# LunaJang/Metabuli_work

Measured on AMD Instinct MI355X. Metric: reads/sec classified (150bp & 10kb) vs GTDB-scale DB at 1/2/4/8 MI355X, higher is better.
Workload: dtype u64

## Files before the change

metabuli_work_amd/classifier.py:

```python
from __future__ import annotations

import ctypes
import dataclasses
import gzip
import os
from typing import Iterator, List, Optional, Tuple

import numpy as np

from . import _abi
from ._abi import KMER_DTYPE, MATCH_DTYPE, RESULT_DTYPE, TAXCNT_DTYPE, MtbParams, ptr
from ._lib import MtbError, check, lib


@dataclasses.dataclass
class LocalParameters:
    seqMode: int = 2
    kmerFormat: int = 1
    syncmer: int = 0
    smerLen: int = 5
    reducedAA: int = 0
    skipRedundancy: int = 0
    minScore: float = 0.0
    minSpScore: float = 0.0
# ... 176 lines not shown
            o1 = off1[lo:hi + 1]
            o2 = off2[lo:hi + 1] if off2 is not None else None
            self.classify_batch(seq1, o1, seq2, o2, device_input=device_input, fetch=False)
            rec = torch.empty((hi - lo, _abi.RESULT_DTYPE.itemsize), dtype=torch.uint8, device=dev)
            self.copy_results(rec.data_ptr(), on_device=True)
            pool = torch.empty((max(self.n_taxcnt(), 1), _abi.TAXCNT_DTYPE.itemsize), dtype=torch.uint8, device=dev)
            nt = self.copy_taxcnt(pool.data_ptr(), on_device=True)
            q, m = self.last_counts()
            recs.append(rec)
            pools.append(pool[:nt])
            qk, mm = qk + q, mm + m
            st = self.stats()
            stats = st if stats is None else {k: (max(stats[k], v) if k == "max_read_matches" else
                                                  v if k in ("join_path", "uniform_units") else stats[k] + v)
                                              for k, v in st.items()}
            stage += self.stage_ms()
            kern += self.kernel_ms()
        recs[1].view(torch.int32).view(-1, _abi.RESULT_DTYPE.itemsize // 4)[:, 4] += pools[0].shape[0]
        torch.cuda.synchronize(dev)
        self._dev_batch = _DevBatch(torch.cat(recs), torch.cat(pools), qk, mm, stats, stage, kern)

    def _classify_halves(self, seq1, off1, seq2, off2, n, device_input) -> BatchResult:
        mid = n // 2
        parts = []
        for lo, hi in ((0, mid), (mid, n)):
            o1 = off1[lo:hi + 1]
            o2 = off2[lo:hi + 1] if off2 is not None else None
            parts.append(self.classify_batch(seq1, o1, seq2, o2, device_input=device_input))
        a, b = parts
        rb = b.results.copy()
        rb["taxcnt_offset"] += len(a.taxcnt)
        return BatchResult(np.concatenate([a.results, rb]), np.concatenate([a.taxcnt, b.taxcnt]),
                           a.query_kmers + b.query_kmers, a.matches + b.matches, a.stage_ms + b.stage_ms)

    def taxcnt(self) -> np.ndarray:
        if getattr(self, "_dev_batch", None) is not None:
            return self._dev_batch.taxcnt.cpu().numpy().reshape(-1).view(TAXCNT_DTYPE).copy()
        nt = ctypes.c_uint64(0)
        lib().mtb_get_taxcnt(self.handle, ctypes.c_void_p(0), 0, ctypes.byref(nt))
        tc = np.zeros(int(nt.value), TAXCNT_DTYPE)
        check(lib().mtb_get_taxcnt(self.handle, ptr(tc), len(tc), ctypes.byref(nt)), "mtb_get_taxcnt")
        return tc

    def last_counts(self) -> Tuple[int, int]:
        if getattr(self, "_dev_batch", None) is not None:
            return self._dev_batch.query_kmers, self._dev_batch.matches
        q, m = ctypes.c_uint64(0), ctypes.c_uint64(0)
        lib().mtb_last_counts(self.handle, ctypes.byref(q), ctypes.byref(m))
        return int(q.value), int(m.value)

    STATS = ["slots", "query_kmers", "matched_queries", "matches", "max_read_matches", "groups", "groups_ge2",
             "species_runs", "wave_runs", "wave_runs_emulated", "join_path", "live_matches", "gallop_queries",
             "spilled_matches", "long_run_queries", "filter_reruns", "db_records_read", "dup_aa_queries",
             "dup_key_queries", "uniform_units"]

    def stats(self) -> dict:
        if getattr(self, "_dev_batch", None) is not None:
            return dict(self._dev_batch.stats)
        out = (ctypes.c_uint64 * len(self.STATS))()
        lib().mtb_last_stats(self.handle, out, len(self.STATS))
        return {k: int(v) for k, v in zip(self.STATS, out)}

    def stage_ms(self) -> np.ndarray:
        if getattr(self, "_dev_batch", None) is not None:
            return self._dev_batch.stage_ms.copy()
        ms = (ctypes.c_float * 5)()
        lib().mtb_last_stage_ms(self.handle, ms, 5)
        return np.array(list(ms), np.float32)

    def kernel_ms(self) -> np.ndarray:
        if getattr(self, "_dev_batch", None) is not None:
            return self._dev_batch.kernel_ms.copy()
        ms = (ctypes.c_float * 7)()
        lib().mtb_last_kernel_ms(self.handle, ms, 7)
        return np.array(list(ms), np.float32)

    def _copy_dev(self, t, dst_ptr: int, on_device: bool) -> None:
        import torch

        del on_device
        if t.numel():
            torch.cuda.synchronize(t.device)
            check(lib().mtb_memcpy(ctypes.c_void_p(dst_ptr), ctypes.c_void_p(t.data_ptr()), t.numel()), "mtb_memcpy")

    def copy_results(self, dst_ptr: int, on_device: bool = True) -> None:
        if getattr(self, "_dev_batch", None) is not None:
            return self._copy_dev(self._dev_batch.results, dst_ptr, on_device)
        check(lib().mtb_copy_results(self.handle, ctypes.c_void_p(dst_ptr), int(on_device)), "mtb_copy_results")

    def n_taxcnt(self) -> int:
        if getattr(self, "_dev_batch", None) is not None:
            return int(self._dev_batch.taxcnt.shape[0])
        nt = ctypes.c_uint64(0)
        lib().mtb_get_taxcnt(self.handle, ctypes.c_void_p(0), 0, ctypes.byref(nt))
        return int(nt.value)

    def copy_taxcnt(self, dst_ptr: int, on_device: bool = True) -> int:
        if getattr(self, "_dev_batch", None) is not None:
            self._copy_dev(self._dev_batch.taxcnt, dst_ptr, on_device)
            return int(self._dev_batch.taxcnt.shape[0])
        nt = ctypes.c_uint64(0)
        check(lib().mtb_copy_taxcnt(self.handle, ctypes.c_void_p(dst_ptr), int(on_device), ctypes.byref(nt)),
              "mtb_copy_taxcnt")
        return int(nt.value)

    def query_kmers(self) -> np.ndarray:
        q = self.stats()["query_kmers"]
# ... 216 lines not shown
```

metabuli_work_amd/csrc/mtb_api.hip:

```cpp
#include <chrono>
#include <cmath>
#include <cstdio>
#include <cstring>
#include <string>
#include <vector>
#include <algorithm>
#include <memory>
#include <charconv>
#include <mutex>
#include <unordered_map>

#include "mtb_host.h"
#include "mtb_launch.h"
#include <cstdlib>

using namespace mtb;

#define HIP_TRY(x)                                                                                   \
    do {                                                                                             \
        hipError_t e_ = (x);                                                                         \
        if (e_ != hipSuccess) {                                                                      \
            set_error(std::string("HIP error ") + hipGetErrorString(e_) + " at " #x);                 \
            return e_ == hipErrorOutOfMemory ? MTB_ERR_OOM : MTB_ERR_HIP;                            \
        }                                                                                            \
// ... 110 lines not shown
    uint64_t binRcForce = 0;
    bool binDigits = true;
    bool uniformUnits = true;
    uint32_t upr = 0;
    uint64_t binHost[kSortBins] = {};
    bool noFilter = false;
    uint32_t spillShift = 0;
    bool sparse = false;
    uint32_t maxW = 0;
    uint32_t maxMate = 0;
    int sortLoFine = kQuerySortLoFine;
    bool forceGeneric = false;
    bool segsortGlobal = false;
    uint32_t mergeSeg = 0;
    int waveTaxon = -1;
    int emulateAll = 0;
    bool pruneCompact = true;
    bool noAlias = false;
    uint64_t aliasBytes = 0;
    int32_t* spOf = nullptr;
    int32_t maxTax = 0;
    int32_t *tNodeOf = nullptr, *tNodeTax = nullptr, *tParent = nullptr, *tDepth = nullptr, *tSpParent = nullptr;
    uint8_t* tFlags = nullptr;
    uint32_t cladePerMatch = 2;
    std::vector<int32_t> hNodeOf;
    std::vector<std::string> hRank;
    HostTaxonomy hTax;
    mutable std::vector<std::string> lineage;
    mutable std::once_flag lineageOnce;
    std::shared_ptr<void> pipelineCache;
    mutable mtb::TaxText taxText;
    mutable std::once_flag taxTextOnce;
    WsBudget ws;
    DevBuf seq1, off1, seq2, off2, meta, reserve, slotOff, qlen, scanTmp;
    DevBuf keysA, valsA, keysB, valsB, radixCounts, radixOffs;
    DevBuf readCnt, mOff, matches, matchesSorted, segScratch, maxSeg, errFlag;
    DevBuf ordKA, ordVA, ordKB, ordVB, matchWin, unitRead, unitInfo, mStage, mRank, mTotal, mDirect, ovFlag, waveList, waveCount, devStats;
    DevBuf qFrom, probeStats;
    DevBuf longList, longCnt;
    DevBuf qStart;
    uint32_t longCap = 0;
    DevBuf chunkIn, chunkCnt, chunkSrcOff;
    DevBuf liveCnt, liveOff;
    DevBuf runFlag, runCnt, runScan;
    DevBuf segLen;
    DevBuf sizeLists;
    DevBuf digA, digB;
    DevBuf binCnt, binTab;
    DevBuf maskOut1, maskOut2, maskProb, maskScale;
    DevBuf readLens;
    DevBuf readCnt64;
    uint64_t liveM = 0;
    double openS[8] = {0, 0, 0, 0, 0, 0, 0, 0};
    static constexpr int kNumStats = 20;
    uint64_t stats[kNumStats] = {};
    uint32_t chunkC = 1;
    uint64_t stageRegion = 0;
    uint64_t spillCap = 0;
    DevBuf emMap, emCnt, emScratch, emPacked, emCnt32, emOff;
    bool emValid = false;
    bool emPackedValid = false;
    std::vector<mtb_em_map> emHost;
    std::vector<uint32_t> spKmers;
    std::string dbDir;
    DevBuf local, paths, comb, conn, spScore, spKeep,
        pathCnt, gStart, sStart, runGroup, clade, tcPool, tcLen, tcOff, tcOut, results;
    uint32_t nReads = 0;
    uint64_t Q = 0, M = 0, nTaxcnt = 0;
    uint64_t Qall = 0;
    double presentShare = 0.5;
    const uint64_t* qKeys = nullptr;
    const uint32_t* qSlots = nullptr;
    bool keepStages = false;
    bool probed = false;
    bool matchOnly = false;
    float stageMs[5] = {0, 0, 0, 0, 0};
    hipEvent_t ev[6]{};
    static constexpr int kNumKern = 7;
    float kernMs[kNumKern] = {0, 0, 0, 0, 0, 0, 0};
    hipEvent_t kev[2 * kNumKern]{};
};

static std::vector<DevBuf*> batch_bufs(mtb_ctx* c);

static void bind_workspace(mtb_ctx* c, size_t cap) {
    c->ws.cap = cap;
    if (const char* e = getenv("MTB_WORKSPACE_CAP")) {
        char* end = nullptr;
        double v = strtod(e, &end);
        const char u = end ? *end : 0;
        v *= u == 'G' || u == 'g' ? 1e9 : u == 'M' || u == 'm' ? 1e6 : u == 'K' || u == 'k' ? 1e3 : 1.0;
        c->ws.cap = v > 0 ? (size_t)v : 0;
    }
    for (DevBuf* b : batch_bufs(c)) b->budget = &c->ws;
}

static void free_db(mtb_ctx* c) {
    if (c->dbArrays) {
        c->dbArrays.reset();
        c->db = nullptr;
        c->dirMem = nullptr;
        c->lines = nullptr;
        c->lineP = nullptr;
        c->runOff = nullptr;
        c->lineExt = nullptr;
        c->link = nullptr;
        return;
// ... 1251 lines not shown
    const uint32_t maxW = metaMax[0];
    c->maxMate = metaMax[1];
    const uint32_t C = std::min<uint32_t>(std::max<uint32_t>(maxW, 1), 64);
    c->maxW = maxW;
    c->upr = c->uniformUnits && maxW <= 64 ? (paired ? 12u : 6u) : 0u;
    c->stats[19] = c->upr;
    launch_read_units(c->meta.as<ReadMeta>(), n, C, c->upr, c->reserve.as<uint32_t>(), s);
    exclusive_scan_u32(c->reserve.as<uint32_t>(), n, c->slotOff.as<uint64_t>(), c->scanTmp.p, s);
    uint64_t U = 0;
    HIP_TRY(hipMemcpyAsync(&U, c->slotOff.as<uint64_t>() + n, sizeof(uint64_t), hipMemcpyDeviceToHost, s));
    HIP_TRY(hipStreamSynchronize(s));
    HIP_TRY(c->unitRead.ensure(sizeof(uint32_t) * std::max<uint64_t>(U, 1)));
    launch_unit_read(c->slotOff.as<uint64_t>(), n, c->unitRead.as<uint32_t>(), s);
    const uint64_t R = extract_slots(U, C);
    const uint64_t Rc = std::max<uint64_t>(R, 1);
    if (R >= 0xFFFFFFFFull) { set_error("batch has >= 2^32 k-mer slots: split it"); return MTB_ERR_ARG; }
    c->chunkC = C;
    c->stats[0] = R;
    c->stats[15] = 0;
    HIP_TRY(c->unitInfo.ensure(16 * std::max<uint64_t>(U, 1)));
    HIP_TRY(c->errFlag.ensure(sizeof(int)));
    HIP_TRY(hipMemsetAsync(c->errFlag.p, 0, sizeof(int), s));
    HIP_TRY(c->mOff.ensure(sizeof(uint64_t) * (n + 1)));
    c->probed = !c->forceGeneric && c->joinMode == 2;
    c->stats[10] = c->probed ? 0 : 1;
    c->matchOnly = (flags & MTB_MATCH_ONLY) != 0;
    int jrc = join_stage(c, dSeq1, dOff1, dSeq2, dOff2, n, U, C, R, Rc);
    if (jrc != MTB_OK) return jrc;
    if (c->matchOnly) {
        for (int k = 10; k < 14; k++) HIP_TRY(hipEventRecord(c->kev[k], s));
        c->nTaxcnt = 0;
    } else {
        int rc = assign_stage(c, n, c->keepStages);
        if (rc != MTB_OK) return rc;
    }
    HIP_TRY(hipEventRecord(c->ev[4], s));
    HIP_TRY(hipGetLastError());
    int err = 0;
    unsigned long long dstat[4] = {0, 0, 0, 0};
    HIP_TRY(hipMemcpyAsync(&err, c->errFlag.p, sizeof(int), hipMemcpyDeviceToHost, s));
    HIP_TRY(hipMemcpyAsync(dstat, c->devStats.p, sizeof(dstat), hipMemcpyDeviceToHost, s));
    if (results && !c->matchOnly)
        HIP_TRY(hipMemcpyAsync(results, c->results.p, sizeof(mtb_result) * n, hipMemcpyDeviceToHost, s));
    HIP_TRY(hipStreamSynchronize(s));
    c->stats[9] = dstat[1];
    {
        std::vector<unsigned long long> ps(kProbeStatsLen);
        HIP_TRY(hipMemcpy(ps.data(), c->probeStats.p, sizeof(unsigned long long) * ps.size(), hipMemcpyDeviceToHost));
        c->stats[2] = 0;
        for (uint32_t i = 0; i < kStatStripes; i++) c->stats[2] += ps[i];
        c->stats[12] = ps[kStatStripes];
        c->stats[16] = 0;
        for (uint32_t i = 0; i < kStatStripes; i++) c->stats[16] += ps[kStatStripes + 1 + i];
    }
    for (int k = 0; k < 4; k++) HIP_TRY(hipEventElapsedTime(&c->stageMs[k], c->ev[k], c->ev[k + 1]));
    HIP_TRY(hipEventElapsedTime(&c->stageMs[4], c->ev[0], c->ev[4]));
    for (int k = 0; k < mtb_ctx::kNumKern; k++)
        HIP_TRY(hipEventElapsedTime(&c->kernMs[k], c->kev[2 * k], c->kev[2 * k + 1]));
    if (const char* e = getenv("MTB_WS_REPORT"); e && atoi(e)) {
        const std::vector<DevBuf*> bufs = batch_bufs(c);
        const char* const* names = batch_buf_names();
        std::vector<std::pair<uint64_t, const char*>> big;
        for (size_t i = 0; i < bufs.size(); i++)
            if (bufs[i]->bytes >= (256ull << 20)) big.push_back({bufs[i]->bytes, names[i]});
        std::sort(big.begin(), big.end(), [](auto& a, auto& b) { return a.first > b.first; });
        fprintf(stderr, "[mtb ws] %u reads, Q %llu, M %llu, live %llu: workspace %.2f GB (K6 scratch aliased %.2f GB):",
                n, (unsigned long long)c->Q, (unsigned long long)c->M, (unsigned long long)c->liveM,
                ctx_workspace_bytes(c) / 1e9, c->aliasBytes / 1e9);
        for (auto& b : big) fprintf(stderr, " %s %.2f", b.second, b.first / 1e9);
        fprintf(stderr, "\n");
    }
    return err ? batch_error(err) : MTB_OK;
}

int mtb_classify_batch(mtb_ctx* c, const char* seq, const uint64_t* off, const char* seq2, const uint64_t* off2,
                       uint32_t n, uint32_t flags, mtb_result* results) {
    const int rc = classify_batch(c, seq, off, seq2, off2, n, flags, results);
    if (rc != MTB_ERR_OOM) return rc;
    (void)hipGetLastError();
    const double held = c->ws.used * 1e-9;
    mtb::ctx_release_workspace(c);
    char msg[200];
    snprintf(msg, sizeof msg, "out of HBM for the workspace of a %u-read batch (%.2f GB held%s): classify it in smaller "
             "pieces", n, held, c->ws.cap ? ", capped" : "");
    set_error(msg);
    return MTB_RETRY;
}

int mtb_get_taxcnt(mtb_ctx* c, mtb_taxcnt* out, uint64_t cap, uint64_t* n_out) {
    if (!c || !n_out) return MTB_ERR_ARG;
    *n_out = c->nTaxcnt;
    if (cap < c->nTaxcnt) return MTB_RETRY;
    if (c->nTaxcnt) HIP_TRY(hipMemcpy(out, c->tcOut.p, sizeof(mtb_taxcnt) * c->nTaxcnt, hipMemcpyDeviceToHost));
    return MTB_OK;
}

int mtb_device_results(mtb_ctx* c, void** results, void** taxcnt, uint64_t* n_taxcnt) {
    if (!c) return MTB_ERR_ARG;
    if (results) *results = c->results.p;
    if (taxcnt) *taxcnt = c->tcOut.p;
    if (n_taxcnt) *n_taxcnt = c->nTaxcnt;
    return MTB_OK;
}

int mtb_last_counts(const mtb_ctx* c, uint64_t* q, uint64_t* m) {
    if (!c) return MTB_ERR_ARG;
// ... 706 lines not shown
```

metabuli_work_amd/csrc/mtb_kernels.hip:

```cpp
#include "mtb_launch.h"

#include <cstring>
#include <type_traits>

namespace mtb {

constexpr int kBlock = 256;
constexpr int kWaves = kBlock / 64;

__device__ __forceinline__ unsigned long long wave_inclusive_scan(unsigned long long x) {
    const int lane = threadIdx.x & 63;
#pragma unroll
    for (int d = 1; d < 64; d <<= 1) {
        unsigned long long y = __shfl_up(x, d, 64);
        if (lane >= d) x += y;
    }
    return x;
}

template <int WAVES = kWaves>
__device__ __forceinline__ unsigned long long block_exclusive_scan(unsigned long long x, unsigned long long* total) {
    __shared__ unsigned long long wsum[WAVES];
    const int lane = threadIdx.x & 63, w = threadIdx.x >> 6;
    unsigned long long inc = wave_inclusive_scan(x);
// ... 1816 lines not shown
                }
                continue;
            }
            SegMatch* out = direct + o;
            if (small[j]) {
                const bool rev = ((info_frame(info[j]) < 3) != (kmerFormat == 2));
                uint64_t wj = rk[j];
#pragma unroll
                for (int k = 0; k < 2; k++)
                    if (rs[j][k] <= thr[j])
                        emit_match(key[j], hr[j], info[j], rv[j][k], rt[j][k], rs[j][k], rev, spOf, maxTax, out,
                                   nullptr, wj++, 0, err);
            } else if (staged) {
                run_emit(key[j], hr[j], info[j], sDb, sInfo, lo[j], hi[j], thr[j], spOf, maxTax, kmerFormat, out,
                         nullptr, rk[j], rk[j] + c[j], 0, err);
            } else {
                run_emit(key[j], hr[j], info[j], dbv, dbtax, lo[j], hi[j], thr[j], spOf, maxTax, kmerFormat, out,
                         nullptr, rk[j], rk[j] + c[j], 0, err);
            }
        }
        return;
    }
    unsigned long long blockTot;
    uint64_t w = block_exclusive_scan(mine, &blockTot);
    const uint32_t reg = blockIdx.x % kStageRegions;
    if (threadIdx.x == 0) sBase = blockTot ? atomicAdd(&total[reg], blockTot) : 0;
    __syncthreads();
    const uint64_t base = sBase;
    if (base + blockTot > region) return;
    w += base + (uint64_t)reg * region;
#pragma unroll
    for (int j = 0; j < kPer; j++) {
        if (!c[j]) continue;
        if (small[j]) {
            const bool rev = ((info_frame(info[j]) < 3) != (kmerFormat == 2));
            uint64_t wj = w;
#pragma unroll
            for (int k = 0; k < 2; k++)
                if (rs[j][k] <= thr[j])
                    emit_match(key[j], hr[j], info[j], rv[j][k], rt[j][k], rs[j][k], rev, spOf, maxTax, buf, bufRank,
                               wj++, rk[j]++, err);
        } else if (staged) {
            run_emit(key[j], hr[j], info[j], sDb, sInfo, lo[j], hi[j], thr[j], spOf, maxTax, kmerFormat, buf, bufRank,
                     w, w + c[j], rk[j], err);
        } else {
            run_emit(key[j], hr[j], info[j], dbv, dbtax, lo[j], hi[j], thr[j], spOf, maxTax, kmerFormat, buf, bufRank,
                     w, w + c[j], rk[j], err);
        }
        w += c[j];
    }
}

constexpr int kWaveLines = 16;
template <bool kExt>
__global__ void __launch_bounds__(256) __attribute__((amdgpu_waves_per_eu(8)))
k_join_uniform(const uint64_t* __restrict__ qkey, const uint32_t* __restrict__ qslot, uint32_t C, uint64_t Q,
               const DbRec* __restrict__ db, uint64_t D, const int32_t* __restrict__ spOf, uint32_t maxTax,
               int kmerFormat, unsigned long long* __restrict__ total, mtb_match* __restrict__ buf,
               uint32_t* __restrict__ bufRank, uint64_t region, int* __restrict__ err,
               const ProbeLine* __restrict__ lines, const uint64_t* __restrict__ lineP,
               const uint16_t* __restrict__ runOff, int sortLo, unsigned long long* __restrict__ stats,
               SegMatch* __restrict__ direct, int* __restrict__ overflow, uint32_t capShift,
               LongRun* __restrict__ longList, uint32_t longCap, uint32_t* __restrict__ longCnt, uint32_t upr,
               unsigned long long* __restrict__ cnt64, const ProbeExt* __restrict__ lineExt) {
    __shared__ uint4 sLineMem[4 * kWaveLines * 4];
    __shared__ uint4 sExtMem[kExt ? 4 * kWaveLines * 4 : 1];
    uint4* const myExt4 = sExtMem + (kExt ? (threadIdx.x >> 6) * kWaveLines * 4 : 0);
    const uint32_t* const myExt = reinterpret_cast<const uint32_t*>(myExt4);
    __shared__ uint64_t sLineP[4 * kWaveLines];
    const int lane = (int)(threadIdx.x & 63), wv = (int)(threadIdx.x >> 6);
    uint4* const myLines = sLineMem + wv * kWaveLines * 4;
    uint64_t* const myLineP = sLineP + wv * kWaveLines;
    const ProbeLine* const sLines = reinterpret_cast<const ProbeLine*>(myLines);
    const DbVal dbv{db};
    const DbTax dbtax{db};
    const int sh = sortLo - 24;
    auto lineSpan = [&](uint64_t kFirst, uint64_t kLast, uint64_t& L0, uint64_t& L1) {
        L0 = ((kFirst >> sortLo) << sh) / kLineRanks;
        L1 = ((((kLast >> sortLo) + 1) << sh) - 1) / kLineRanks;
    };
    auto join = [&](const uint64_t q, const bool live, const uint64_t key, const uint32_t slot, const uint64_t L0,
                    const bool inLds, const uint32_t tile) {
        uint64_t lo = 0, hi = 0;
        bool gallop = false;
        if (live) {
            const uint64_t aa = key & kAAMask, x = aa >> 24, L = x / kLineRanks;
            const uint32_t o = (uint32_t)(x - L * kLineRanks);
            const ProbeLine* pl = inLds ? sLines + (L - L0) : lines + L;
            uint32_t before, pc;
            bool present;
            const uint64_t head = line_scan(pl, o, before, pc, present);
            const uint64_t base = head & ((1ull << 40) - 1), cnt = head >> 40;
            if (cnt > kRunIdxMax) {
                gallop = true;
                lo = gallop_lower1(dbv, base + before, aa);
                hi = gallop_lower1(dbv, lo, aa + (1ull << 24));
            } else if (present) {
                uint32_t sum = 0, code = 0;
                if (kExt && inLds && before < kExtRanks && ext_run_rolled(myExt + (L - L0) * (kExtRanks / 16), before, sum, code)) {
                    lo = base + before + sum;
                    hi = lo + code + 1;
                } else {
                    const uint64_t p = (inLds ? myLineP[L - L0] : lineP[L]) + before;
                    const uint32_t a = runOff[p], b1 = runOff[p + 1];
                    lo = base + a;
                    hi = base + (before + 1 < pc ? b1 : (uint32_t)cnt);
                }
            } else {
                lo = hi = base;
            }
            if (lo > D) {
                atomicExch(err, kErrRunOutsideDb);
                lo = D;
            }
            if (hi > D - 1) hi = D - 1;
            if (lo > hi) hi = lo;
        }
        const uint64_t n = hi - lo;
        const bool longq = n > kLongRun;
        const bool small = live && n <= 2;
        uint64_t v0 = 0, v1 = 0;
        uint32_t t0 = 0, t1 = 0;
        if (small && n) {
            const DbRec r0 = db[lo], r1 = n == 2 ? db[lo + 1] : DbRec{0, 0, 0};
            v0 = (uint64_t)r0.hi << 32 | r0.lo;
            v1 = (uint64_t)r1.hi << 32 | r1.lo;
            t0 = r0.tax;
            t1 = r1.tax;
        }
        const HamRows hr = hamming_rows(key);
        uint32_t c = 0, thr = 0, s0 = 255, s1 = 255;
        if (small) {
            s0 = n > 0 ? hamming_sum_rows(hr, v0) : 255u;
            s1 = n > 1 ? hamming_sum_rows(hr, v1) : 255u;
            thr = min(min(s0, s1) * 2u, 7u);
            c = (uint32_t)(s0 <= thr) + (uint32_t)(s1 <= thr);
        } else if (live && !longq) {
            c = run_select(hr, dbv, 0, lo, hi, D, thr);
        }
        const bool e0 = small && s0 <= thr, e1 = small && s1 <= thr;
        const int32_t sp0 = e0 ? (t0 <= maxTax ? spOf[t0] : 0) : 0;
        const int32_t sp1 = e1 ? (t1 <= maxTax ? spOf[t1] : 0) : 0;
        uint32_t rk = 0, r = 0;
        uint64_t info = 0;
        if (c) {
            uint32_t p;
            const uint32_t u = slot_unit(slot, C, p);
            r = u / upr;
            const unsigned long long old = atomicAdd(&cnt64[r], (unsigned long long)c);
            rk = (uint32_t)old;
            info = uniform_unit_info(u, p, upr, (uint32_t)(old >> 32), kmerFormat);
        }
        const uint64_t lm = __ballot(longq && live);
        if (lm) {
            uint32_t at = 0;
            if (lane == 0) at = atomicAdd(longCnt, (uint32_t)__popcll(lm));
            at = (uint32_t)__shfl((int)at, 0, 64) + (uint32_t)__popcll(lm & ((1ull << lane) - 1));
            if (longq && live && at < longCap) longList[at] = LongRun{q, lo, hi};
        }
        const uint64_t hw = __ballot(c != 0);
        if (lane == 0 && hw) atomicAdd(&stats[tile % kStatStripes], (unsigned long long)__popcll(hw));
        const uint64_t gw = __ballot(gallop);
        if (gw && (threadIdx.x & 63) == 0) atomicAdd(&stats[kStatStripes], (unsigned long long)__popcll(gw));
        if (!c) return;
        const bool rev = ((info_frame(info) < 3) != (kmerFormat == 2));
        const uint64_t cap = ((uint64_t)upr * C) >> capShift;
        const bool spill = rk + c > cap;
        uint64_t w = rk;
        if (spill) {
            const uint64_t sp = atomicAdd(&total[0], (unsigned long long)c);
            if (sp + c > region) {
                atomicExch(overflow, 1);
                return;
            }
            w = sp;
        }
        SegMatch* const out = direct + (uint64_t)r * upr * C;
        if (small) {
    #pragma unroll
            for (int k = 0; k < 2; k++) {
                if (!(k ? e1 : e0)) continue;
                const uint64_t tv = k ? v1 : v0;
                const uint32_t tax = k ? t1 : t0, hs = k ? s1 : s0;
                const int32_t sp = k ? sp1 : sp0;
                if (tax == 0 || sp <= 0) atomicExch(err, kErrTaxid);
                mtb_match m;
                m.qinfo = info;
                m.target_id = tax;
                m.species_id = (uint32_t)sp;
                m.dna_encoding = (uint32_t)(tv & 0xFFFFFFull);
                m.right_end_hamming = (uint16_t)hammings_rows(hr, key, tv, rev);
                m.hamming = (uint8_t)hs;
                m.pad = 0;
                if (spill) {
                    bufRank[w] = rk++;
                    buf[w] = m;
                } else {
                    out[w] = seg_pack(m);
                }
                w++;
            }
        } else if (spill) {
            run_emit(key, hr, info, dbv, dbtax, lo, hi, thr, spOf, maxTax, kmerFormat, buf, bufRank, w, w + c, rk, err);
        } else {
            run_emit(key, hr, info, dbv, dbtax, lo, hi, thr, spOf, maxTax, kmerFormat, out, (uint32_t*)nullptr, w, w + c, 0,
                     err);
        }
    };
    const uint64_t waveId = ((uint64_t)blockIdx.x * blockDim.x + threadIdx.x) >> 6;
    const uint64_t q0 = waveId * 64;
    if (q0 >= Q) return;
    const uint64_t q1 = min(q0 + 64, Q);
    const uint64_t q = q0 + (uint64_t)lane;
    const bool live = q < q1;
    const uint64_t key = live ? qkey[q] : 0;
    const uint32_t slot = live ? qslot[q] : 0;
    uint64_t L0, L1;
    lineSpan((uint64_t)__shfl((long long)key, 0, 64), (uint64_t)__shfl((long long)key, (int)(q1 - q0 - 1), 64), L0, L1);
    const bool inLds = L1 - L0 < (uint64_t)kWaveLines;
    if (inLds) {
        const uint32_t nv = (uint32_t)(L1 - L0 + 1) * 4;
        const uint4* src = reinterpret_cast<const uint4*>(lines + L0);
        uint4 v{0, 0, 0, 0}, xv{0, 0, 0, 0};
        uint64_t lp = 0;
        if ((uint32_t)lane < nv) v = src[lane];
        if (kExt && (uint32_t)lane < nv) xv = reinterpret_cast<const uint4*>(lineExt + L0)[lane];
        if ((uint32_t)lane <= (uint32_t)(L1 - L0)) lp = lineP[L0 + lane];
        if ((uint32_t)lane < nv) myLines[lane] = v;
        if (kExt && (uint32_t)lane < nv) myExt4[lane] = xv;
        if ((uint32_t)lane <= (uint32_t)(L1 - L0)) myLineP[lane] = lp;
        __builtin_amdgcn_s_waitcnt(0);
        __builtin_amdgcn_wave_barrier();
    }
    join(q, live, key, slot, L0, inLds, (uint32_t)waveId);
}

__global__ void __launch_bounds__(64) k_match_long(const LongRun* __restrict__ list, const uint64_t* __restrict__ qkey,
                                                   const uint32_t* __restrict__ qslot,
                                                   const uint64_t* __restrict__ unitInfo, uint32_t C,
                                                   const DbRec* __restrict__ db, uint64_t D,
                                                   const int32_t* __restrict__ spOf, uint32_t maxTax, int kmerFormat,
                                                   uint32_t* __restrict__ readCnt,
                                                   unsigned long long* __restrict__ total, mtb_match* __restrict__ buf,
                                                   uint32_t* __restrict__ bufRank, uint64_t region, int* __restrict__ err,
                                                   SegMatch* __restrict__ direct, const uint64_t* __restrict__ dirOff,
                                                   int* __restrict__ overflow, uint32_t capShift,
                                                   unsigned long long* __restrict__ stats,
                                                   unsigned long long* __restrict__ cnt64) {
    const LongRun lr = list[blockIdx.x];
    if (lr.lo > lr.hi || lr.hi > D - 1) {
        if (threadIdx.x == 0) atomicExch(err, kErrRunOutsideDb);
// ... 602 lines not shown
    const uint64_t q = (uint64_t)blockIdx.x * 256 + threadIdx.x;
    sk[threadIdx.x] = q < Q ? qkey[q] : ~0ull;
    __syncthreads();
    for (uint32_t k = 2; k <= 256; k <<= 1)
        for (uint32_t j = k >> 1; j > 0; j >>= 1) {
            const uint32_t i = threadIdx.x, l = i ^ j;
            if (l > i) {
                const uint64_t a = sk[i], b = sk[l];
                if (((i & k) == 0) == (a > b)) {
                    sk[i] = b;
                    sk[l] = a;
                }
            }
            __syncthreads();
        }
    const uint32_t i = threadIdx.x;
    const bool valid = sk[i] != ~0ull && i > 0;
    const uint32_t aa = valid && (sk[i] >> 24) == (sk[i - 1] >> 24), same = valid && sk[i] == sk[i - 1];
    const int nAa = __syncthreads_count(aa), nSame = __syncthreads_count(same);
    if (threadIdx.x == 0) {
        if (nAa) atomicAdd(&out[0], (unsigned long long)nAa);
        if (nSame) atomicAdd(&out[1], (unsigned long long)nSame);
    }
}

void launch_dup_stats(const uint64_t* qkey, uint64_t Q, unsigned long long* out, hipStream_t s) {
    if (Q) k_dup_stats<<<(unsigned)((Q + 255) / 256), 256, 0, s>>>(qkey, Q, out);
}

uint64_t match_window_elems(uint64_t Q) { return 2 * ((Q + kMatchQ - 1) / kMatchQ); }

void launch_match_windows(const uint64_t* qkey, uint64_t Q, const DbRec* db, uint64_t D, const AADir& dir,
                          int kmerFormat, uint64_t* win, hipStream_t s) {
    if (Q == 0 || D < 2) return;
    const uint64_t nb = (Q + kMatchQ - 1) / kMatchQ;
    k_match_windows<<<(unsigned)((2 * nb + 255) / 256), 256, 0, s>>>(qkey, Q, db, D, dir, kmerFormat, nb, win);
}

void launch_match(const uint64_t* qkey, const uint32_t* qslot, const uint64_t* unitInfo, uint32_t C, uint64_t Q,
                  const DbRec* db, uint64_t D, const AADir& dir, const int32_t* spOf,
                  uint32_t maxTax, int kmerFormat, uint32_t* readCnt, unsigned long long* total, mtb_match* buf,
                  uint32_t* bufRank, uint64_t region, int* err, uint32_t winCap, const uint64_t* win,
                  const ProbeLine* lines, const uint64_t* lineP, const uint16_t* runOff, int sortLo,
                  unsigned long long* stats, SegMatch* direct, const uint64_t* dirOff, int* overflow,
                  uint32_t capShift, LongRun* longList, uint32_t longCap, uint32_t* longCnt, hipStream_t s,
                  const ProbeExt* lineExt, uint32_t upr, unsigned long long* cnt64) {
    if (Q == 0 || D < 2) return;
    winCap = std::min<uint32_t>(winCap, kMatchWin);
    if (unstaged_join(lines != nullptr, D, Q, winCap)) {
        const unsigned blocks = (unsigned)((Q + 256 * kFreePer - 1) / (256 * kFreePer));
        const char* fe = getenv("MTB_JOIN_FAST");
        const bool fastOk = (!fe || atoi(fe) != 0) && lines && runOff && direct && longList && upr && cnt64;
        const bool ext = runOff && lineExt;
        if (fastOk && ext)
            k_join_uniform<true><<<(unsigned)((Q + 255) / 256), 256, 0, s>>>(
                qkey, qslot, C, Q, db, D, spOf, maxTax, kmerFormat, total, buf, bufRank, region, err, lines, lineP, runOff,
                sortLo, stats, direct, overflow, capShift, longList, longCap, longCnt, upr, cnt64, lineExt);
        else if (fastOk)
            k_join_uniform<false><<<(unsigned)((Q + 255) / 256), 256, 0, s>>>(
                qkey, qslot, C, Q, db, D, spOf, maxTax, kmerFormat, total, buf, bufRank, region, err, lines, lineP, runOff,
                sortLo, stats, direct, overflow, capShift, longList, longCap, longCnt, upr, cnt64, nullptr);
        else if (ext)
            k_match<false, false><<<blocks, 256, 0, s>>>(qkey, qslot, unitInfo, C, Q, db, D, dir, spOf, maxTax, kmerFormat,
                                                         readCnt, total, buf, bufRank, region, err, winCap, win, lines,
                                                         lineP, runOff, sortLo, stats, direct, dirOff, overflow, capShift,
                                                         longList, longCap, longCnt, lineExt, upr, cnt64);
        else
            k_match<false, true><<<blocks, 256, 0, s>>>(qkey, qslot, unitInfo, C, Q, db, D, dir, spOf, maxTax, kmerFormat,
                                                        readCnt, total, buf, bufRank, region, err, winCap, win, lines,
                                                        lineP, runOff, sortLo, stats, direct, dirOff, overflow, capShift,
                                                        longList, longCap, longCnt, nullptr, upr, cnt64);
    } else {
        const unsigned blocks = (unsigned)((Q + kMatchQ - 1) / kMatchQ);
        k_match<true, false><<<blocks, 256, 0, s>>>(qkey, qslot, unitInfo, C, Q, db, D, dir, spOf,
                                                            maxTax, kmerFormat, readCnt, total, buf, bufRank, region,
                                                            err, winCap, win, lines, nullptr, nullptr, kQuerySortLo,
                                                            stats, direct, dirOff, overflow, capShift, nullptr, 0,
                                                            longCnt, nullptr, upr, cnt64);
    }
}

__global__ void __launch_bounds__(256) k_compact_segments(const SegMatch* __restrict__ in,
                                                          const uint64_t* __restrict__ dirOff, uint32_t C,
                                                          const uint64_t* __restrict__ readOff, uint32_t nReads,
                                                          mtb_match* __restrict__ out, uint32_t capShift, int mode) {
    const uint32_t r = blockIdx.x * 4 + (threadIdx.x >> 6), lane = threadIdx.x & 63;
    if (r >= nReads) return;
    const uint64_t src = dirOff[r] * C, dst = readOff[r];
    const uint64_t cap = ((dirOff[r + 1] - dirOff[r]) * C) >> capShift;
    const bool over = readOff[r + 1] - dst > cap;
    if ((mode == 1 && !over) || (mode == 2 && over)) return;
    const uint64_t n = min(readOff[r + 1] - dst, cap);
    for (uint64_t i = lane; i < n; i += 64) out[dst + i] = seg_expand(in[src + i], (uint64_t)(r + 1) << 32);
}

__global__ void k_spill_scatter(const mtb_match* __restrict__ spill, const uint32_t* __restrict__ spillRank,
                                const unsigned long long* __restrict__ total, const uint64_t* __restrict__ readOff,
                                uint32_t nReads, mtb_match* __restrict__ out, int* __restrict__ err) {
    const uint64_t i = (uint64_t)blockIdx.x * blockDim.x + threadIdx.x;
    if (i >= total[0]) return;
    const mtb_match m = spill[i];
    const uint32_t r = info_seq(m.qinfo) - 1;
    if (r >= nReads || readOff[r] + spillRank[i] >= readOff[r + 1]) {
        atomicExch(err, kErrStagedRead);
        return;
    }
    out[readOff[r] + spillRank[i]] = m;
}

void launch_spill_scatter(const mtb_match* spill, const uint32_t* spillRank, const unsigned long long* total,
                          uint64_t nSpill, const uint64_t* readOff, uint32_t nReads, mtb_match* out, int* err,
                          hipStream_t s) {
    if (nSpill) k_spill_scatter<<<(unsigned)((nSpill + 255) / 256), 256, 0, s>>>(spill, spillRank, total, readOff, nReads,
                                                                               out, err);
// ... 512 lines not shown
```

metabuli_work_amd/csrc/mtb_launch.h:

```cpp
#pragma once
#include <hip/hip_runtime.h>
#include <stdint.h>

#include <utility>

#include "mtb_device.h"

namespace mtb {

constexpr int kErrTaxid = 1;
constexpr int kErrStagedRead = 2;
constexpr int kErrProbeStash = 3;
constexpr int kErrProbeCount = 4;
constexpr int kErrRunOutsideDb = 5;
constexpr int kErrLiveCount = 6;

struct ReadMeta {
    int32_t len1, len2, ql1, ql2, w1, w2;
};

struct HostTables {
    uint8_t base[256];
    int8_t aa[64];
    int8_t num[64];
// ... 65 lines not shown
uint64_t extract_slots(uint64_t nUnits, uint32_t C);
void launch_extract(const uint8_t* seq1, const uint64_t* off1, const uint8_t* seq2, const uint64_t* off2,
                    const ReadMeta* meta, const uint64_t* uOff, const uint32_t* unitRead, uint64_t nUnits,
                    uint32_t C, const HostTables& t, int kmerFormat, int syncmer, int smerLen, uint64_t* keys,
                    uint64_t* unitInfo, hipStream_t s, uint32_t upr = 0);

uint64_t radix_counts_elems(uint64_t n);
template <typename V>
uint64_t radix_sort_pairs(uint64_t* keysA, V* valsA, uint64_t* keysB, V* valsB, uint64_t n, int bitLo, int bitHi,
                          bool filter, bool genVals, uint32_t* counts, uint64_t* offs, void* scanTmp, bool* inB,
                          hipStream_t s, uint8_t* digA = nullptr, uint8_t* digB = nullptr, bool unstableFirst = false);
constexpr int kSortBins = 2048;
uint64_t radix_binned_tiles(const uint64_t* binHost, uint64_t rc);
template <typename V>
uint64_t radix_sort_binned(uint64_t* keysR, V* valsR, uint64_t* keysT, V* valsT, const uint64_t* binHost,
                           const unsigned long long* binDev, uint64_t rc, int bitLo, int bitHi, uint32_t* counts,
                           uint64_t* offs, void* scanTmp, uint64_t* tileTab, bool* inT, hipStream_t s, uint8_t* digR,
                           uint8_t* digT);
void launch_to_rank_form(uint64_t* v, uint64_t n, hipStream_t s);
uint64_t host_from_rank_form(uint64_t v);
constexpr uint64_t kAARankEnd = 37822859361ull;
constexpr int kQuerySortLo = 36, kQuerySortHi = 60;
constexpr int kQuerySortLoFine = 36;

uint64_t decode_diff_chunk(const uint16_t* diff, uint64_t n, uint64_t carry, uint64_t* values, uint32_t* flagTmp,
                           uint64_t* idxTmp, void* scanTmp, uint64_t* lastTerm, uint64_t* lastValue, hipStream_t s);
void launch_mask_info(uint32_t* info, uint64_t n, uint32_t mask, hipStream_t s);

struct DbRec {
    uint32_t lo, hi, tax;
};
static_assert(sizeof(DbRec) == 12, "12-B DB records");
void launch_pack_db(const uint64_t* v, const uint32_t* tax, uint64_t n, DbRec* out, hipStream_t s);
void launch_rec_rank_form(DbRec* db, uint64_t n, hipStream_t s);
void launch_rec_mask_info(DbRec* db, uint64_t n, uint32_t mask, hipStream_t s);

struct AADir {
    const uint64_t* dir;
    uint64_t R;
    uint64_t div;
    int L;
    int fmt;
};
AADir make_aa_dir(uint64_t D, int kmerFormat);
void build_aa_dir(const DbRec* db, uint64_t D, const AADir& d, uint64_t* dir, hipStream_t s);

constexpr uint32_t kLineRanks = 448;
struct alignas(64) ProbeLine {
    uint64_t base;
    uint32_t bits[kLineRanks / 32];
};
static_assert(sizeof(ProbeLine) == 64, "one probe line per 64-B segment");
constexpr uint32_t kStatStripes = 256;
constexpr uint32_t kProbeStatsLen = 2 * kStatStripes + 1;
constexpr uint64_t kDbPad = 8;
constexpr uint64_t kProbeLines = (kAARankEnd + kLineRanks - 1) / kLineRanks + 1;
void build_probe_lines(const DbRec* db, uint64_t D, const AADir& dir, ProbeLine* lines,
                       hipStream_t s);

constexpr uint64_t kRunIdxMax = 0xFFFF;
void build_line_prefix(const ProbeLine* lines, uint64_t* lineP, uint32_t* popTmp, void* scanTmp, hipStream_t s);
void build_run_offsets(const DbRec* db, uint64_t D, const ProbeLine* lines, const uint64_t* lineP,
                       uint16_t* runOff, hipStream_t s);
constexpr uint32_t kExtRanks = 256;
struct alignas(64) ProbeExt {
    uint32_t w[kExtRanks / 16];
};
static_assert(sizeof(ProbeExt) == 64, "one run-length line per probe line");
void build_line_ext(const ProbeLine* lines, const uint64_t* lineP, const uint16_t* runOff, ProbeExt* ext,
                    hipStream_t s);
void launch_line_ext_check(const ProbeLine* lines, const uint64_t* lineP, const uint16_t* runOff, const ProbeExt* ext,
                           unsigned long long* out, hipStream_t s);

constexpr uint64_t kLinkSlots = 1801088541ull;
static_assert(kLinkSlots * 21 == kAARankEnd, "21^8 AA ranks");
void build_link_lines(const ProbeLine* lines, uint64_t* link, hipStream_t s);
void launch_link_check(const ProbeLine* lines, const uint64_t* link, unsigned long long* out, hipStream_t s);

uint64_t launch_extract_filter(const uint8_t* seq1, const uint64_t* off1, const uint8_t* seq2, const uint64_t* off2,
                               const ReadMeta* meta, const uint64_t* uOff, const uint32_t* unitRead, uint64_t nUnits,
                               uint32_t C, const HostTables& t, int kmerFormat, int syncmer, int smerLen,
                               uint64_t* unitInfo, const ProbeLine* lines, uint64_t* qkey, uint32_t* qslot,
                               unsigned long long* counter, uint64_t rankLo, uint64_t rankHi, uint64_t* emitted,
                               uint64_t cap, bool threadMajor, hipStream_t s,
                               uint8_t* qdig = nullptr, unsigned long long* binCnt = nullptr, uint64_t binRc = 0,
                               uint64_t* binHost = nullptr, uint32_t upr = 0, const uint64_t* link = nullptr,
                               bool seqFits = true);
uint64_t launch_filter(const uint64_t* keys, uint64_t R, const ProbeLine* lines, uint64_t* qkey, uint32_t* qslot,
                       uint64_t* qfrom, unsigned long long* counter, uint64_t rankLo, uint64_t rankHi,
                       uint64_t* emitted, hipStream_t s);
void launch_probe(const uint64_t* qkey, const uint32_t* qslot, const uint64_t* qfrom, uint64_t Q,
                  const uint64_t* unitInfo, uint32_t C, const DbRec* db, uint64_t D,
                  const int32_t* spOf, uint32_t maxTax, int kmerFormat, uint32_t* readCnt, unsigned long long* total,
                  mtb_match* buf, uint32_t* bufRank, uint64_t region, int* err, unsigned long long* stats,
                  hipStream_t s);

constexpr uint32_t kSegMaxTax = (1u << 24) - 1;
struct SegMatch {
    uint32_t posFrame, targetHam, speciesReh, dnaReh;
};
static_assert(sizeof(SegMatch) == 16, "16-B segment matches");
__host__ __device__ inline SegMatch seg_pack(const mtb_match& m) {
    return SegMatch{(uint32_t)m.qinfo | (uint32_t)(m.qinfo >> 61) << 29, m.target_id | (uint32_t)m.hamming << 24,
                    m.species_id | (uint32_t)(m.right_end_hamming & 0xFFu) << 24,
                    (m.dna_encoding & 0xFFFFFFu) | (uint32_t)(m.right_end_hamming >> 8) << 24};
}
__host__ __device__ inline mtb_match seg_expand(const SegMatch& s, uint64_t seqBits) {
// ... 131 lines not shown
```

Baseline: 35.07 million.

## Keep uniform-join runs up to four records in registers and tally longer runs

The uniform join kernel is templated on a register run length R (default 4, selectable through MTB_JOIN_REG_RUN). Runs of up to R records are loaded into lane registers and matches are written straight from packed fields, replacing the two-record special case. Longer non-long runs now use a per-lane loop with an 8-bit histogram of Hamming sums instead of run_select. New per-wave counters for looped queries are added to the probe stats. This enlarges the fast in-register path, at the cost of more registers per lane and a per-lane serial loop that may diverge within a wave.

```diff
diff --git a/metabuli_work_amd/classifier.py b/metabuli_work_amd/classifier.py
--- a/metabuli_work_amd/classifier.py
+++ b/metabuli_work_amd/classifier.py
@@ -252,7 +252,7 @@
     STATS = ["slots", "query_kmers", "matched_queries", "matches", "max_read_matches", "groups", "groups_ge2",
              "species_runs", "wave_runs", "wave_runs_emulated", "join_path", "live_matches", "gallop_queries",
              "spilled_matches", "long_run_queries", "filter_reruns", "db_records_read", "dup_aa_queries",
-             "dup_key_queries", "uniform_units"]
+             "dup_key_queries", "uniform_units", "loop_queries", "loop_waves"]
 
     def stats(self) -> dict:
         if getattr(self, "_dev_batch", None) is not None:
diff --git a/metabuli_work_amd/csrc/mtb_api.hip b/metabuli_work_amd/csrc/mtb_api.hip
--- a/metabuli_work_amd/csrc/mtb_api.hip
+++ b/metabuli_work_amd/csrc/mtb_api.hip
@@ -186,7 +186,7 @@
     DevBuf readCnt64;
     uint64_t liveM = 0;
     double openS[8] = {0, 0, 0, 0, 0, 0, 0, 0};
-    static constexpr int kNumStats = 20;
+    static constexpr int kNumStats = 22;
     uint64_t stats[kNumStats] = {};
     uint32_t chunkC = 1;
     uint64_t stageRegion = 0;
@@ -1544,6 +1544,11 @@
         c->stats[12] = ps[kStatStripes];
         c->stats[16] = 0;
         for (uint32_t i = 0; i < kStatStripes; i++) c->stats[16] += ps[kStatStripes + 1 + i];
+        c->stats[20] = c->stats[21] = 0;
+        for (uint32_t i = 0; i < kStatStripes; i++) {
+            c->stats[20] += ps[kLoopStats + i];
+            c->stats[21] += ps[kLoopStats + kStatStripes + i];
+        }
     }
     for (int k = 0; k < 4; k++) HIP_TRY(hipEventElapsedTime(&c->stageMs[k], c->ev[k], c->ev[k + 1]));
     HIP_TRY(hipEventElapsedTime(&c->stageMs[4], c->ev[0], c->ev[4]));
diff --git a/metabuli_work_amd/csrc/mtb_kernels.hip b/metabuli_work_amd/csrc/mtb_kernels.hip
--- a/metabuli_work_amd/csrc/mtb_kernels.hip
+++ b/metabuli_work_amd/csrc/mtb_kernels.hip
@@ -1892,7 +1892,8 @@
 }
 
 constexpr int kWaveLines = 16;
-template <bool kExt>
+constexpr int kJoinRegRun = 4;
+template <bool kExt, int R>
 __global__ void __launch_bounds__(256) __attribute__((amdgpu_waves_per_eu(8)))
 k_join_uniform(const uint64_t* __restrict__ qkey, const uint32_t* __restrict__ qslot, uint32_t C, uint64_t Q,
                const DbRec* __restrict__ db, uint64_t D, const int32_t* __restrict__ spOf, uint32_t maxTax,
@@ -1958,38 +1959,65 @@
         }
         const uint64_t n = hi - lo;
         const bool longq = n > kLongRun;
-        const bool small = live && n <= 2;
-        uint64_t v0 = 0, v1 = 0;
-        uint32_t t0 = 0, t1 = 0;
-        if (small && n) {
-            const DbRec r0 = db[lo], r1 = n == 2 ? db[lo + 1] : DbRec{0, 0, 0};
-            v0 = (uint64_t)r0.hi << 32 | r0.lo;
-            v1 = (uint64_t)r1.hi << 32 | r1.lo;
-            t0 = r0.tax;
-            t1 = r1.tax;
+        const bool lane_run = live && !longq;
+        const bool small = lane_run && n <= (uint64_t)R;
+        const bool loopq = lane_run && n > (uint64_t)R;
+        uint32_t dna[R], tax[R];
+#pragma unroll
+        for (int k = 0; k < R; k++) {
+            const DbRec rec = lane_run && (uint64_t)k < n ? db[lo + k] : DbRec{0, 0, 0};
+            dna[k] = rec.lo;
+            tax[k] = rec.tax;
         }
         const HamRows hr = hamming_rows(key);
-        uint32_t c = 0, thr = 0, s0 = 255, s1 = 255;
+        uint32_t pu;
+        const uint32_t u = slot_unit(slot, C, pu);
+        const uint32_t r = u / upr, local = u - r * upr;
+        const bool rev = (((local >= 6u ? local - 6u : local) < 3u) != (kmerFormat == 2));
+        uint32_t wTax[R], wDna[R], rehLo = 0, minSum = 255;
+#pragma unroll
+        for (int k = 0; k < R; k++) {
+            const uint32_t s = lane_run && (uint64_t)k < n ? hamming_sum_rows(hr, dna[k]) : 255u;
+            minSum = min(minSum, s);
+            wTax[k] = (tax[k] & kSegMaxTax) | s << 24;
+            wDna[k] = 0;
+        }
+        uint32_t c = 0, thr = min(minSum * 2u, 7u), sel = 0;
         if (small) {
-            s0 = n > 0 ? hamming_sum_rows(hr, v0) : 255u;
-            s1 = n > 1 ? hamming_sum_rows(hr, v1) : 255u;
-            thr = min(min(s0, s1) * 2u, 7u);
-            c = (uint32_t)(s0 <= thr) + (uint32_t)(s1 <= thr);
-        } else if (live && !longq) {
-            c = run_select(hr, dbv, 0, lo, hi, D, thr);
-        }
-        const bool e0 = small && s0 <= thr, e1 = small && s1 <= thr;
-        const int32_t sp0 = e0 ? (t0 <= maxTax ? spOf[t0] : 0) : 0;
-        const int32_t sp1 = e1 ? (t1 <= maxTax ? spOf[t1] : 0) : 0;
-        uint32_t rk = 0, r = 0;
+#pragma unroll
+            for (int k = 0; k < R; k++) {
+                if ((wTax[k] >> 24) > thr) continue;
+                sel |= 1u << k;
+                const uint32_t reh = hammings_rows(hr, key, dna[k], rev);
+                wDna[k] = (dna[k] & 0xFFFFFFu) | (reh >> 8) << 24;
+                rehLo |= (reh & 0xFFu) << (8 * k);
+            }
+            c = (uint32_t)__popc(sel);
+        }
+        int32_t sp[R];
+#pragma unroll
+        for (int k = 0; k < R; k++) sp[k] = (sel >> k & 1u) && tax[k] <= maxTax ? spOf[tax[k]] : 0;
+        if (loopq) {
+            uint64_t tally = 0;
+#pragma unroll
+            for (int k = 0; k < R; k++)
+                if ((wTax[k] >> 24) <= 7u) tally += 1ull << (8 * (wTax[k] >> 24));
+            for (uint64_t t = lo + R; t < hi; t++) {
+                const uint32_t s = hamming_sum_rows(hr, dbv[t]);
+                minSum = min(minSum, s);
+                if (s <= 7) tally += 1ull << (8 * s);
+            }
+            thr = min(minSum * 2u, 7u);
+#pragma unroll
+            for (uint32_t s = 0; s < 8; s++)
+                if (s <= thr) c += (uint32_t)(tally >> (8 * s)) & 0xFFu;
+        }
+        uint32_t rk = 0;
         uint64_t info = 0;
         if (c) {
-            uint32_t p;
-            const uint32_t u = slot_unit(slot, C, p);
-            r = u / upr;
             const unsigned long long old = atomicAdd(&cnt64[r], (unsigned long long)c);
             rk = (uint32_t)old;
-            info = uniform_unit_info(u, p, upr, (uint32_t)(old >> 32), kmerFormat);
+            info = uniform_unit_info(u, pu, upr, (uint32_t)(old >> 32), kmerFormat);
         }
         const uint64_t lm = __ballot(longq && live);
         if (lm) {
@@ -2002,8 +2030,12 @@
         if (lane == 0 && hw) atomicAdd(&stats[tile % kStatStripes], (unsigned long long)__popcll(hw));
         const uint64_t gw = __ballot(gallop);
         if (gw && (threadIdx.x & 63) == 0) atomicAdd(&stats[kStatStripes], (unsigned long long)__popcll(gw));
+        const uint64_t lw = __ballot(loopq);
+        if (lane == 0 && lw) {
+            atomicAdd(&stats[kLoopStats + tile % kStatStripes], (unsigned long long)__popcll(lw));
+            atomicAdd(&stats[kLoopStats + kStatStripes + tile % kStatStripes], 1ull);
+        }
         if (!c) return;
-        const bool rev = ((info_frame(info) < 3) != (kmerFormat == 2));
         const uint64_t cap = ((uint64_t)upr * C) >> capShift;
         const bool spill = rk + c > cap;
         uint64_t w = rk;
@@ -2017,26 +2049,25 @@
         }
         SegMatch* const out = direct + (uint64_t)r * upr * C;
         if (small) {
-    #pragma unroll
-            for (int k = 0; k < 2; k++) {
-                if (!(k ? e1 : e0)) continue;
-                const uint64_t tv = k ? v1 : v0;
-                const uint32_t tax = k ? t1 : t0, hs = k ? s1 : s0;
-                const int32_t sp = k ? sp1 : sp0;
-                if (tax == 0 || sp <= 0) atomicExch(err, kErrTaxid);
-                mtb_match m;
-                m.qinfo = info;
-                m.target_id = tax;
-                m.species_id = (uint32_t)sp;
-                m.dna_encoding = (uint32_t)(tv & 0xFFFFFFull);
-                m.right_end_hamming = (uint16_t)hammings_rows(hr, key, tv, rev);
-                m.hamming = (uint8_t)hs;
-                m.pad = 0;
+            const uint32_t posFrame = (uint32_t)info | (uint32_t)(info >> 61) << 29;
+#pragma unroll
+            for (int k = 0; k < R; k++) {
+                if (!(sel >> k & 1u)) continue;
+                const uint32_t t = wTax[k] & kSegMaxTax, lowReh = rehLo >> (8 * k) & 0xFFu;
+                if (t == 0 || sp[k] <= 0) atomicExch(err, kErrTaxid);
                 if (spill) {
+                    mtb_match m;
+                    m.qinfo = info;
+                    m.target_id = t;
+                    m.species_id = (uint32_t)sp[k];
+                    m.dna_encoding = wDna[k] & 0xFFFFFFu;
+                    m.right_end_hamming = (uint16_t)(lowReh | (wDna[k] >> 24) << 8);
+                    m.hamming = (uint8_t)(wTax[k] >> 24);
+                    m.pad = 0;
                     bufRank[w] = rk++;
                     buf[w] = m;
                 } else {
-                    out[w] = seg_pack(m);
+                    out[w] = SegMatch{posFrame, wTax[k], (uint32_t)sp[k] | lowReh << 24, wDna[k]};
                 }
                 w++;
             }
@@ -2745,14 +2776,26 @@
         const char* fe = getenv("MTB_JOIN_FAST");
         const bool fastOk = (!fe || atoi(fe) != 0) && lines && runOff && direct && longList && upr && cnt64;
         const bool ext = runOff && lineExt;
+        int regRun = kJoinRegRun;
+        if (const char* re = getenv("MTB_JOIN_REG_RUN")) {
+            const int v = atoi(re);
+            if (v >= 2 && v <= 4) {
+                regRun = v;
+            } else {
+                static bool told = false;
+                if (!told) fprintf(stderr, "[mtb] MTB_JOIN_REG_RUN=%s is not 2, 3 or 4: using %d\n", re, kJoinRegRun);
+                told = true;
+            }
+        }
+        auto joinUniform = [&](auto kernel) {
+            kernel<<<(unsigned)((Q + 255) / 256), 256, 0, s>>>(
+                qkey, qslot, C, Q, db, D, spOf, maxTax, kmerFormat, total, buf, bufRank, region, err, lines, lineP, runOff,
+                sortLo, stats, direct, overflow, capShift, longList, longCap, longCnt, upr, cnt64, ext ? lineExt : nullptr);
+        };
         if (fastOk && ext)
-            k_join_uniform<true><<<(unsigned)((Q + 255) / 256), 256, 0, s>>>(
-                qkey, qslot, C, Q, db, D, spOf, maxTax, kmerFormat, total, buf, bufRank, region, err, lines, lineP, runOff,
-                sortLo, stats, direct, overflow, capShift, longList, longCap, longCnt, upr, cnt64, lineExt);
+            joinUniform(regRun == 2 ? k_join_uniform<true, 2> : regRun == 3 ? k_join_uniform<true, 3> : k_join_uniform<true, 4>);
         else if (fastOk)
-            k_join_uniform<false><<<(unsigned)((Q + 255) / 256), 256, 0, s>>>(
-                qkey, qslot, C, Q, db, D, spOf, maxTax, kmerFormat, total, buf, bufRank, region, err, lines, lineP, runOff,
-                sortLo, stats, direct, overflow, capShift, longList, longCap, longCnt, upr, cnt64, nullptr);
+            joinUniform(regRun == 2 ? k_join_uniform<false, 2> : regRun == 3 ? k_join_uniform<false, 3> : k_join_uniform<false, 4>);
         else if (ext)
             k_match<false, false><<<blocks, 256, 0, s>>>(qkey, qslot, unitInfo, C, Q, db, D, dir, spOf, maxTax, kmerFormat,
                                                          readCnt, total, buf, bufRank, region, err, winCap, win, lines,
diff --git a/metabuli_work_amd/csrc/mtb_launch.h b/metabuli_work_amd/csrc/mtb_launch.h
--- a/metabuli_work_amd/csrc/mtb_launch.h
+++ b/metabuli_work_amd/csrc/mtb_launch.h
@@ -141,7 +141,8 @@
 };
 static_assert(sizeof(ProbeLine) == 64, "one probe line per 64-B segment");
 constexpr uint32_t kStatStripes = 256;
-constexpr uint32_t kProbeStatsLen = 2 * kStatStripes + 1;
+constexpr uint32_t kLoopStats = 2 * kStatStripes + 1;
+constexpr uint32_t kProbeStatsLen = 4 * kStatStripes + 1;
 constexpr uint64_t kDbPad = 8;
 constexpr uint64_t kProbeLines = (kAARankEnd + kLineRanks - 1) / kLineRanks + 1;
 void build_probe_lines(const DbRec* db, uint64_t D, const AADir& dir, ProbeLine* lines,
```

Result: faster. 36.38 million (median of 6 runs) (+3.7%).
